# BVE-Reborn/rend3

Hardware: NVIDIA H100
Metric: culled objects/s (fused frustum cull + object-uniform bake) (higher is better)
Workload: dtype f32

## Files before the change

### include/rend3_b200.h

```cpp
#ifndef REND3_B200_H
#define REND3_B200_H

#include <stddef.h>
#include <stdint.h>

#include "r3_layouts.h"

#ifdef __cplusplus
extern "C" {
#endif

#define R3_ABI_VERSION 1u
#define R3_MAX_SHADOWS 63u

enum {
    R3_OK = 0,
    R3_E_INVALID = -1,
    R3_E_CUDA = -2,
    R3_E_OOM = -3,
    R3_E_NO_DEVICE = -4,
    R3_E_STATE = -5
};

typedef struct r3_ctx r3_ctx;

uint32_t r3_abi_version(void);
int r3_ctx_create(int device, r3_ctx** out);
int r3_ctx_destroy(r3_ctx* ctx);
const char* r3_last_error(const r3_ctx* ctx);
int r3_sync(r3_ctx* ctx);
int r3_get_stream(r3_ctx* ctx, void** stream);
int r3_launch_count(r3_ctx* ctx, uint64_t* launches);

int r3_frame_begin(r3_ctx* ctx);
int r3_frame_end(r3_ctx* ctx);
int r3_frame_graph_stats(r3_ctx* ctx, uint64_t stats[4]);

int r3_set_stage_timing(r3_ctx* ctx, int enabled);
int r3_stage_times(r3_ctx* ctx, double ms[8], uint32_t launches[8]);

int r3_set_objects(r3_ctx*, const r3_object* records, uint32_t n_slots);
int r3_update_objects(r3_ctx*, const uint32_t* slots, const r3_object* records, uint32_t n);
int r3_set_objects_device(r3_ctx*, const void* device_records, uint32_t n_slots);
int r3_set_object_sort_info(r3_ctx*, const uint64_t* material_key, const uint8_t* flags,
                            const float* location_xyz, uint32_t n_slots);
int r3_update_object_sort_info(r3_ctx*, const uint32_t* slots, const uint64_t* material_key, const uint8_t* flags,
                               const float* location_xyz, uint32_t n);
int r3_resize_objects(r3_ctx*, uint32_t n_slots);
int r3_set_object_mesh_spheres(r3_ctx*, const uint32_t* slots_or_null, const float* center_radius , uint32_t n);
int r3_set_object_transforms(r3_ctx*, const uint32_t* slots_or_null, const float* mat4s , uint32_t n);
int r3_set_object_transforms_device(r3_ctx*, const uint32_t* d_slots_or_null, const float* d_mat4s, uint32_t n);
int r3_set_objects_enabled(r3_ctx*, const uint32_t* slots_or_null, const uint8_t* enabled, uint32_t n);
int r3_set_objects_enabled_device(r3_ctx*, const uint32_t* d_slots_or_null, const uint8_t* d_enabled, uint32_t n);
int r3_set_object_variants(r3_ctx*, const r3_object_variant* variants, uint32_t n_variants, const r3_variant_group* groups, uint32_t n_groups,
                           const uint32_t* slots, const uint32_t* slot_groups, uint32_t n_listed);
int r3_switch_object_variants(r3_ctx*, const uint32_t* slots_or_null, const uint32_t* choices, uint32_t n);
int r3_switch_object_variants_device(r3_ctx*, const uint32_t* d_slots_or_null, const uint32_t* d_choices, uint32_t n);
int r3_readback_object_variants(r3_ctx*, uint32_t* out, uint32_t first, uint32_t n);
int r3_set_mesh_buffer(r3_ctx*, const void* bytes, uint64_t nbytes);
int r3_set_deformable_meshes(r3_ctx*, const r3_deformable_mesh* meshes, uint32_t n_meshes,
                             const uint32_t* object_slots, const uint32_t* object_meshes, uint32_t n_objects);
int r3_deform_meshes(r3_ctx*, const float* positions, uint64_t n_floats);
int r3_deform_meshes_device(r3_ctx*, const float* d_positions, uint64_t n_floats);
int r3_readback_deformable_mesh_spheres(r3_ctx*, float* out , uint32_t first, uint32_t n);
int r3_set_remeshable_meshes(r3_ctx*, const r3_remeshable_mesh* meshes, uint32_t n_meshes,
                             const uint32_t* object_slots, const uint32_t* object_meshes, uint32_t n_objects);
int r3_remesh_meshes(r3_ctx*, const uint32_t* counts, const float* positions, const uint32_t* indices, const float* normals,
                     const float* tangents, const float* uv0, const uint32_t* color0, uint64_t n_vertices, uint64_t n_indices);
int r3_remesh_meshes_device(r3_ctx*, const uint32_t* d_counts, const float* d_positions, const uint32_t* d_indices, const float* d_normals,
// ... 126 lines not shown
```

### include/rend3_b200.hpp

```cpp
#ifndef REND3_B200_HPP
#define REND3_B200_HPP

#include <array>
#include <cstdint>
#include <stdexcept>
#include <string>
#include <vector>

#include "rend3_b200.h"

namespace r3 {

struct Error : std::runtime_error {
    int code;
    Error(int c, const std::string& what) : std::runtime_error(what), code(c) {}
};

enum class SampleCount : uint32_t { One = 1, Four = 4 };
enum class CullingSource { Predicted, Residual };

struct CameraSpecifier {
    uint32_t index;
    static CameraSpecifier Viewport() { return {R3_CAMERA_VIEWPORT}; }
    static CameraSpecifier Shadow(uint32_t i) { return {i}; }
// ... 136 lines not shown
class HiZRoutine {
public:
    void add_hi_z_to_graph(Renderer& r) const { r.check(r3_hiz_build(r.raw())); }
};

class TonemappingRoutine {
public:
    void add_to_graph(Renderer& r, bool target_is_srgb) const { r.check(r3_tonemap(r.raw(), target_is_srgb ? 1 : 0)); }
};

class BaseRenderGraph {
public:
    GpuCuller gpu_culler;
    GpuSkinner gpu_skinner;
    ForwardRoutine forward;
    HiZRoutine hi_z;
    TonemappingRoutine tonemapping;
    bool submit_as_graph = false;
    bool device_shadow_cameras = false;
    bool device_point_lights = false;

    void add_to_graph(Renderer& r, const EvalOutput& ev, uint32_t width, uint32_t height, SampleCount samples, const BaseRenderGraphSettings& settings,
                      bool target_is_srgb = true) {
        r.check(r3_set_render_target(r.raw(), width, height, (uint32_t)samples, settings.clear_color.data()));
        if (submit_as_graph) r.check(r3_frame_begin(r.raw()));
        r.check(r3_clear_shadow_atlas(r.raw()));
        r.check(r3_set_frame_uniforms(r.raw(), &ev.uniforms));
        if (device_shadow_cameras) r.check(r3_evaluate_shadow_cameras(r.raw(), ev.viewport_location));
        if (device_point_lights) r.check(r3_evaluate_point_lights(r.raw()));
        if (ev.n_material_updates) r.check(r3_update_materials(r.raw(), ev.material_indices, ev.material_records, ev.n_material_updates));
        if (ev.n_d_material_updates) r.check(r3_update_materials_device(r.raw(), ev.d_material_indices, ev.d_material_records, ev.n_d_material_updates));
        gpu_skinner.add_skinning_to_graph(r, ev);
        for (uint32_t i = 0; i < ev.shadows.size(); ++i) {
            if (device_shadow_cameras) r.check(r3_shadow_uniform_upload(r.raw(), i, ev.n_slots, R3_CB_BAKE | R3_CB_CULL));
            else gpu_culler.object_uniform_upload(r, CameraSpecifier::Shadow(i), ev.shadows[i].header);
        }
        for (uint32_t i = 0; i < ev.shadows.size(); ++i) gpu_culler.add_culling_to_graph(r, CameraSpecifier::Shadow(i), ev.viewport_location);
        for (uint32_t i = 0; i < ev.shadows.size(); ++i) forward.add_shadow_to_graph(r, i, ev.shadows[i]);
        gpu_culler.object_uniform_upload(r, CameraSpecifier::Viewport(), ev.viewport);
        r.check(r3_forward_begin(r.raw()));
        forward.add_forward_to_graph(r, CullingSource::Predicted);
        hi_z.add_hi_z_to_graph(r);
        gpu_culler.add_culling_to_graph(r, CameraSpecifier::Viewport(), ev.viewport_location);
        forward.add_forward_to_graph(r, CullingSource::Residual);
        forward.resolve(r);
        forward.add_transparent_to_graph(r);
        tonemapping.add_to_graph(r, target_is_srgb);
        if (submit_as_graph) r.check(r3_frame_end(r.raw()));
    }
};

}
#endif
```

### rend3_b200/backend.py

```python
from __future__ import annotations

import ctypes as C
import os
from typing import Optional

import numpy as np

from .layouts import (
    BATCH_DTYPE,
    CAMERA_HEADER_DTYPE,
    INDIRECT_CALL_DTYPE,
    OBJECT_MATRICES_DTYPE,
    REGION_DTYPE,
)

CAMERA_VIEWPORT = 0xFFFFFFFF
CB_BAKE, CB_CULL = 1, 2

_ROOT = os.path.dirname(os.path.abspath(__file__))
CUDA_LIB_PATH = os.path.join(_ROOT, "librend3_b200.so")

ENTRY_POINTS = [
    "abi_version", "ctx_create", "ctx_destroy", "last_error", "sync", "get_stream", "launch_count", "set_stage_timing", "stage_times", "frame_begin", "frame_end", "frame_graph_stats",
    "set_objects", "update_objects", "set_objects_device", "set_object_sort_info", "set_mesh_buffer", "set_textures", "set_skybox",
    "set_materials", "set_directional_lights", "set_point_lights", "set_frame_uniforms",
    "object_uniform_upload", "visible_count", "readback_visible", "readback_object_matrices",
    "batch_objects", "batch_counts", "readback_batches", "batching_info", "cull", "readback_indices",
    "readback_draw_calls", "readback_culling_results", "set_render_target", "clear_shadow_atlas",
    "shadow_pass", "forward_begin", "forward_pass", "hiz_build", "forward_resolve", "forward_blend", "tonemap",
    "set_parity_target", "readback_hdr_f32", "readback_hdr_f16", "readback_depth", "readback_ldr", "readback_shadow_atlas",
    "readback_hiz", "forward_stats", "forward_light_evaluations", "device_ptr", "set_scissor_rows", "skin", "readback_mesh_buffer",
    "exchange_create", "exchange_connect", "exchange_words", "exchange_merge", "exchange_merged", "exchange_count", "exchange_counts", "exchange_destroy",
    "peer_create", "peer_connect", "peer_send_atlas_rect", "peer_send_rows", "peer_signal", "peer_wait", "peer_destroy", "clear_shadow_rect", "set_cull_shard",
    "update_object_sort_info", "resize_objects", "update_mesh_buffer", "update_textures",
    "set_animations", "set_skeletons", "set_pose_jobs", "pose_skeletons", "skin_posed", "readback_joint_matrices",
    "set_object_animations", "set_object_pose_jobs", "pose_objects", "readback_objects",
    "set_object_mesh_spheres", "set_object_transforms", "set_object_transforms_device",
    "set_objects_enabled", "set_objects_enabled_device",
    "update_materials", "update_materials_device", "readback_materials",
    "set_joint_matrices", "set_joint_matrices_device",
    "set_deformable_meshes", "deform_meshes", "deform_meshes_device", "readback_deformable_mesh_spheres",
    "set_remeshable_meshes", "remesh_meshes", "remesh_meshes_device", "readback_remesh_status", "debug_invocation_bound",
    "set_object_variants", "switch_object_variants", "switch_object_variants_device", "readback_object_variants",
]


class _AnimLibrary(C.Structure):
    _fields_ = [("skins", C.c_void_p), ("n_skins", C.c_uint32), ("joints", C.c_void_p), ("n_joints", C.c_uint32), ("order", C.c_void_p),
                ("clips", C.c_void_p), ("n_clips", C.c_uint32), ("channels", C.c_void_p), ("n_channels", C.c_uint32),
                ("keys", C.c_void_p), ("n_keys", C.c_uint64)]


class _AnimObjectLibrary(C.Structure):
    _fields_ = [("nodes", C.c_void_p), ("n_nodes", C.c_uint32), ("clips", C.c_void_p), ("n_clips", C.c_uint32), ("channels", C.c_void_p),
                ("n_channels", C.c_uint32), ("keys", C.c_void_p), ("n_keys", C.c_uint64), ("left_handed", C.c_uint32)]


class R3Error(RuntimeError):
    def __init__(self, code: int, message: str):
        super().__init__(f"rend3_b200 error {code}: {message}")
        self.code = code


def _ptr(a: Optional[np.ndarray]):
    return None if a is None else a.ctypes.data_as(C.c_void_p)


def _u32_list(a, what: str) -> np.ndarray:
    a = np.asarray(a)
    assert a.ndim == 1 and a.dtype.kind in "iu", f"{what}: a 1-d integer array"
    assert not len(a) or (a.min() >= 0 and a.max() <= 0xFFFFFFFF), f"{what}: out of the uint32 range"
    return np.ascontiguousarray(a, dtype=np.uint32)


class Backend:

    def __init__(self, lib: C.CDLL, prefix: str = "r3_", device: int = 0):
        self.lib, self.prefix = lib, prefix
        self.ctx = C.c_void_p()
        self._fn("last_error").restype = C.c_char_p
        self._fn("abi_version").restype = C.c_uint32
        rc = self._fn("ctx_create")(C.c_int(device), C.byref(self.ctx))
        if rc != 0:
            raise R3Error(rc, "context creation failed (no CUDA device?)")

    def _fn(self, name):
        return getattr(self.lib, self.prefix + name)

    def _call(self, name, *args):
        rc = self._fn(name)(self.ctx, *args)
        if rc != 0:
            raise R3Error(rc, (self._fn("last_error")(self.ctx) or b"?").decode())

    def close(self):
        if self.ctx:
            self._fn("ctx_destroy")(self.ctx)
            self.ctx = C.c_void_p()

    def __del__(self):
        try:
            self.close()
        except Exception:
            pass

    def sync(self):
        self._call("sync")

    def stream(self) -> int:
        s = C.c_void_p()
        self._call("get_stream", C.byref(s))
        return s.value or 0

    def launch_count(self) -> int:
        n = C.c_uint64()
        self._call("launch_count", C.byref(n))
        return n.value

    STAGES = ("triangle_test", "raster_setup_colour", "raster_setup_depth", "raster_bands", "resolve", "sort", "cull_bake", "triangle_compact")

    def frame_begin(self):
        self._call("frame_begin")

    def frame_end(self):
        self._call("frame_end")

    def frame_graph_stats(self):
        s = (C.c_uint64 * 4)()
        self._call("frame_graph_stats", s)
        return {"frames": int(s[0]), "graphed": int(s[1]), "flushed": int(s[2]), "instantiations": int(s[3])}

    def set_stage_timing(self, enabled: bool = True):
        self._call("set_stage_timing", C.c_int(1 if enabled else 0))

    def stage_times(self):
        ms, n = (C.c_double * 8)(), (C.c_uint32 * 8)()
        self._call("stage_times", ms, n)
        return {name: {"ms": float(ms[i]), "launches": int(n[i])} for i, name in enumerate(self.STAGES)}

    def set_objects(self, records: np.ndarray):
        records = np.ascontiguousarray(records)
        assert records.dtype.itemsize == 128
        self._call("set_objects", _ptr(records), C.c_uint32(len(records)))

    def set_objects_device(self, device_ptr: int, n_slots: int):
        self._call("set_objects_device", C.c_void_p(device_ptr), C.c_uint32(n_slots))

    def update_objects(self, slots: np.ndarray, records: np.ndarray):
        slots = np.ascontiguousarray(slots, dtype=np.uint32)
        records = np.ascontiguousarray(records)
        self._call("update_objects", _ptr(slots), _ptr(records), C.c_uint32(len(slots)))

    def set_object_sort_info(self, material_key, flags, location):
        k = np.ascontiguousarray(material_key, dtype=np.uint64)
        f = np.ascontiguousarray(flags, dtype=np.uint8)
        l = np.ascontiguousarray(location, dtype=np.float32).reshape(-1)
        assert len(f) == len(k) and len(l) == 3 * len(k)
        self._call("set_object_sort_info", _ptr(k), _ptr(f), _ptr(l), C.c_uint32(len(k)))
# ... 664 lines not shown
```

### rend3_b200/csrc/r3_common.cuh

```cuda
#pragma once
#include <cuda_runtime.h>
#include <stdint.h>

#include <string>
#include <vector>

#include "../../include/rend3_b200.h"

#define R3_EXPORT extern "C" __attribute__((visibility("default")))

constexpr int R3_MAX_CAMERAS = 64;

struct r3_iobuf {
    uint8_t* d = nullptr;
    uint64_t capacity_elements = 0, out_elems = 0, in_elems = 0, elem_size = 0;
    bool flipped = false, clear_on_swap = false, created = false;
    uint64_t out_off() const { return flipped ? capacity_elements / 2 : 0; }
    uint64_t in_off() const { return flipped ? 0 : capacity_elements / 2; }
};

struct r3_jobs {
    r3_batch_data* d_batches = nullptr; uint32_t batches_cap = 0, n_batches = 0;
    r3_region* d_regions = nullptr; uint32_t regions_cap = 0, n_regions = 0;
    uint32_t* d_region_first_inv = nullptr;
    uint32_t* d_header = nullptr;
    uint32_t total_invocations = 0;
    bool device_built = false;
    std::vector<r3_batch_data> batches;
    std::vector<r3_region> regions;
    bool valid = false;
};

enum { R3_STAGE_TRIANGLE_TEST = 0, R3_STAGE_RASTER_SETUP_COLOUR, R3_STAGE_RASTER_SETUP_DEPTH, R3_STAGE_RASTER_BANDS, R3_STAGE_RESOLVE, R3_STAGE_SORT,
       R3_STAGE_CULL_BAKE, R3_STAGE_TRIANGLE_COMPACT, R3_STAGE_COUNT };
struct r3_stage_timer {
    bool enabled = false;
    std::vector<cudaEvent_t> pool;
    std::vector<int> stage_of;
    size_t used = 0;
};
constexpr int R3_MAX_EXCHANGE_RANKS = 16;
constexpr int R3_EXCHANGE_SLOTS = 4;
constexpr uint32_t R3_PEER_KINDS = 4;
struct r3_peer_state {
// ... 9 lines not shown
struct r3_camera {
    bool header_set = false;
    r3_camera_header header{};
    r3_object_matrices* d_matrices = nullptr; uint32_t matrices_cap = 0;
    uint32_t* d_visible = nullptr; uint32_t visible_cap = 0;
    uint32_t* d_visible_count = nullptr;
    unsigned long long* d_tile_state = nullptr; uint32_t tile_state_cap = 0;
    uint32_t* d_words = nullptr; uint32_t words_set = 0;
    uint32_t* d_gathered = nullptr; uint32_t ex_ranks = 0, ex_rank = 0, ex_words_per_rank = 0; bool ex_connected = false;
    uint32_t* ex_peers[R3_MAX_EXCHANGE_RANKS] = {};
    uint32_t ex_epoch = 0, ex_objects = 0; uint32_t* d_ex_done = nullptr;
    cudaEvent_t ex_cull_done[R3_EXCHANGE_SLOTS] = {}, ex_merge_done[R3_EXCHANGE_SLOTS] = {}; bool ex_merge_pending[R3_EXCHANGE_SLOTS] = {}; uint32_t ex_consumed[R3_EXCHANGE_SLOTS] = {};
    uint32_t* d_global_visible = nullptr; uint64_t global_visible_cap = 0; uint32_t* d_merge_counts = nullptr; uint64_t merge_counts_cap = 0;
    int visible_count_host = -1;
    r3_jobs jobs[2]; int cur = 0;
    int batching_path = 0;
    uint64_t gsort_epoch_used = ~0ull;
    bool has_draw_call_set = false; int cache_idx = -1;
    std::vector<uint32_t> prev_invocation;
    uint32_t* d_prev_inv[2] = {nullptr, nullptr}; uint32_t prev_inv_cap = 0; int prev_inv_cur = 0;
    unsigned long long* d_sort_keys[2] = {nullptr, nullptr}; uint64_t sort_keys_cap = 0, sort_keys_cap2 = 0;
    uint32_t* d_sort_hist = nullptr; uint64_t sort_hist_cap = 0;
    uint32_t* d_batch_tmp = nullptr; uint64_t batch_tmp_cap = 0;
    r3_iobuf index_buffer, draw_call_buffer, results_buffer;
    uint32_t* d_resid_bits = nullptr; uint64_t resid_bits_cap = 0;
    unsigned long long* d_word_scan = nullptr; uint64_t word_scan_cap = 0;
    unsigned long long* d_block_sums = nullptr; uint64_t block_sums_cap = 0;
};

struct r3_anim_state;
struct r3_deform_state;
struct r3_variant_state;

struct r3_tri_record { float xyw[3][3]; uint32_t object_id; uint32_t vid[3]; uint32_t _pad[3]; };
static_assert(sizeof(r3_tri_record) == 64, "triangle record");

struct r3_ctx {
    int device = 0;
    cudaStream_t stream = nullptr;
    cudaStream_t side_stream = nullptr;
    std::string err;
    uint64_t launches = 0;
    bool coop_launch_ok = false;
    int sm_count = 1;
    r3_object* d_objects = nullptr; uint32_t n_slots = 0, objects_cap = 0; bool objects_borrowed = false;
    float4* d_hot_xyz = nullptr; float4* d_hot_w = nullptr; float4* d_hot_sphere = nullptr; uint32_t* d_enabled_bits = nullptr; uint32_t* d_affine_bits = nullptr;
    float* d_hot_radius = nullptr; uint32_t* d_centre_bits = nullptr;
    uint64_t hot_cap = 0; bool hot_valid = false;
    std::vector<uint64_t> sort_key; std::vector<uint8_t> sort_flags; std::vector<float> sort_loc;
    uint32_t* d_live_bits = nullptr; uint32_t live_bits_cap = 0; bool have_live = false;
    uint8_t* d_sort_key8 = nullptr; float* d_sort_loc = nullptr; uint32_t sort_dev_cap = 0; bool gpu_batching_ok = false;
    float4* d_mesh_spheres = nullptr; uint32_t n_mesh_spheres = 0, mesh_spheres_cap = 0;
    bool locations_moved = false;
    uint32_t sort_live_blend = 0, sort_wide_keys = 0;
    uint32_t sort_blend_slots = 0;
    bool presence_on_device = false;
    bool variants_on_device = false, variant_key2 = false, variant_wide_key = false;
    unsigned long long* d_gsort_keys[2] = {nullptr, nullptr}; uint64_t gsort_cap[2] = {0, 0}; uint32_t* d_gsort_hist = nullptr; uint64_t gsort_hist_cap = 0;
    uint32_t* d_gsort_header = nullptr; int gsort_src = 0; uint32_t gsort_n = 0; bool gsort_valid = false; float gsort_loc[3] = {0, 0, 0};
    uint64_t gsort_epoch = 0, gsort_sorted_epoch = ~0ull; uint32_t gsort_cameras_this_epoch = 0, gsort_cameras_last_epoch = 0;
    uint64_t max_total_invocations = 0, max_object_invocations = 0; bool max_invocations_valid = false;
    uint32_t* d_invocation_floor = nullptr; uint32_t n_invocation_floor = 0, invocation_floor_cap = 0;
    uint32_t* d_mesh = nullptr; uint64_t mesh_words = 0, mesh_cap = 0;
    r3_material* d_materials = nullptr; uint32_t n_materials = 0, materials_cap = 0;
    bool has_skybox = false; r3_texture_desc sky_desc{}; uint8_t* d_sky_texels = nullptr; uint64_t sky_cap = 0;
    r3_texture_desc* d_tex_descs = nullptr; uint32_t n_textures = 0, tex_descs_cap = 0; uint8_t* d_texels = nullptr; uint64_t texels_cap = 0, texel_bytes = 0;
    r3_directional_light* d_dir = nullptr; uint32_t n_dir = 0, dir_cap = 0;
    r3_directional_light_source* d_light_src = nullptr; r3_camera_header* d_shadow_cams = nullptr;
    std::vector<r3_directional_light_source> light_src;
    bool light_src_set = false, shadow_cams_evaluated = false; uint32_t light_src_left_handed = 0;
    uint8_t* d_point = nullptr; uint64_t point_bytes_cap = 0; uint32_t point_capacity = 0;
    r3_point_light_source* d_point_src = nullptr; uint8_t* d_point_live = nullptr; uint32_t point_handles = 0, point_src_cap = 0, point_live_cap = 0;
// ... 156 lines not shown
```

### rend3_b200/csrc/r3_ctx.cu

```cuda
#include <algorithm>
#include <cstdio>
#include <cstdlib>
#include <cstring>
#include <new>

#include "r3_common.cuh"

int r3_fail(r3_ctx* c, int code, const char* msg) {
    if (c) c->err = msg;
    return code;
}
int r3_cuda_fail(r3_ctx* c, cudaError_t e, const char* where) {
    if (c) {
        c->err = std::string(where) + ": " + cudaGetErrorString(e);
    }
    cudaGetLastError();
    return e == cudaErrorMemoryAllocation ? R3_E_OOM : R3_E_CUDA;
}

int r3_reserve(r3_ctx* c, void** ptr, uint64_t* cap, uint64_t need, size_t elem, bool keep, bool zero_new) {
    if (*ptr && *cap >= need) return R3_OK;
    uint64_t ncap = need < 16 ? 16 : need;
    void* n = nullptr;
    R3_CUDA(c, cudaMalloc(&n, ncap * elem));
    if (zero_new) R3_CUDA(c, cudaMemsetAsync(n, 0, ncap * elem, c->stream));
    if (*ptr) {
        if (keep && *cap) R3_CUDA(c, cudaMemcpyAsync(n, *ptr, *cap * elem, cudaMemcpyDeviceToDevice, c->stream));
        R3_CUDA(c, r3_stream_sync(c));
        cudaFree(*ptr);
    }
    *ptr = n;
    *cap = ncap;
    return R3_OK;
}

R3_EXPORT uint32_t r3_abi_version(void) { return R3_ABI_VERSION; }

R3_EXPORT int r3_ctx_create(int device, r3_ctx** out) {
    if (!out) return R3_E_INVALID;
    *out = nullptr;
    int count = 0;
    cudaError_t e = cudaGetDeviceCount(&count);
    if (e != cudaSuccess || count == 0 || device < 0 || device >= count) {
        cudaGetLastError();
        return R3_E_NO_DEVICE;
    }
    r3_ctx* c = new (std::nothrow) r3_ctx();
    if (!c) return R3_E_OOM;
    c->device = device;
    int prio_least = 0, prio_greatest = 0;
    if (cudaSetDevice(device) == cudaSuccess) cudaDeviceGetStreamPriorityRange(&prio_least, &prio_greatest);
    if (cudaSetDevice(device) != cudaSuccess || cudaStreamCreateWithPriority(&c->stream, cudaStreamNonBlocking, prio_greatest) != cudaSuccess) {
        delete c;
        cudaGetLastError();
        return R3_E_CUDA;
    }
    { int coop = 0; cudaDeviceGetAttribute(&coop, cudaDevAttrCooperativeLaunch, device); c->coop_launch_ok = coop != 0; }
    if (cudaDeviceGetAttribute(&c->sm_count, cudaDevAttrMultiProcessorCount, device) != cudaSuccess || c->sm_count < 1) { cudaStreamDestroy(c->stream); delete c; cudaGetLastError(); return R3_E_CUDA; }
    if (cudaMalloc((void**)&c->d_stats, 8 * sizeof(unsigned long long)) != cudaSuccess) { delete c; return R3_E_OOM; }
    cudaMemsetAsync(c->d_stats, 0, 64, c->stream);
    c->point_bytes_cap = 16 + 16 * sizeof(r3_point_light);
    if (cudaMalloc((void**)&c->d_point, c->point_bytes_cap) != cudaSuccess) { cudaFree(c->d_stats); delete c; return R3_E_OOM; }
    cudaMemsetAsync(c->d_point, 0, c->point_bytes_cap, c->stream);
    *out = c;
    return R3_OK;
}

static void free_jobs(r3_jobs& j) { cudaFree(j.d_batches); cudaFree(j.d_regions); cudaFree(j.d_region_first_inv); cudaFree(j.d_header); }

R3_EXPORT int r3_ctx_destroy(r3_ctx* c) {
    if (!c) return R3_E_INVALID;
    cudaSetDevice(c->device);
    r3_stream_sync(c);
    if (c->side_stream) cudaStreamSynchronize(c->side_stream);
    r3_peer_destroy(c);
    r3_anim_destroy(c);
    r3_deform_destroy(c);
    r3_variants_destroy(c);
    if (!c->objects_borrowed) cudaFree(c->d_objects);
    cudaFree(c->d_hot_xyz); cudaFree(c->d_hot_w); cudaFree(c->d_hot_sphere); cudaFree(c->d_enabled_bits); cudaFree(c->d_affine_bits); cudaFree(c->d_hot_radius); cudaFree(c->d_centre_bits); cudaFree(c->d_tex_descs); cudaFree(c->d_texels); cudaFree(c->d_sky_texels);
    cudaFree(c->d_sort_key8); cudaFree(c->d_sort_loc); cudaFree(c->d_gsort_keys[0]); cudaFree(c->d_gsort_keys[1]); cudaFree(c->d_gsort_hist); cudaFree(c->d_gsort_header);
    cudaFree(c->d_mesh_spheres); cudaFree(c->d_live_bits); cudaFree(c->d_mesh); cudaFree(c->d_materials); cudaFree(c->d_dir); cudaFree(c->d_point);
    cudaFree(c->d_light_mats); cudaFree(c->d_atlas); cudaFree(c->d_light_src); cudaFree(c->d_shadow_cams); cudaFree(c->d_point_src); cudaFree(c->d_point_live);
    for (auto& k : c->cams) {
        cudaFree(k.d_matrices); cudaFree(k.d_visible); cudaFree(k.d_visible_count); cudaFree(k.d_tile_state);
        if (k.d_gathered) {
            for (uint32_t r = 0; r < k.ex_ranks; ++r)
                if (k.ex_connected && r != k.ex_rank && k.ex_peers[r]) cudaIpcCloseMemHandle(k.ex_peers[r]);
            cudaFree(k.d_gathered);
        }
        cudaFree(k.d_ex_done); cudaFree(k.d_global_visible); cudaFree(k.d_merge_counts);
        for (int q = 0; q < R3_EXCHANGE_SLOTS; ++q) { if (k.ex_cull_done[q]) cudaEventDestroy(k.ex_cull_done[q]); if (k.ex_merge_done[q]) cudaEventDestroy(k.ex_merge_done[q]); }
        free_jobs(k.jobs[0]); free_jobs(k.jobs[1]);
        cudaFree(k.index_buffer.d); cudaFree(k.draw_call_buffer.d); cudaFree(k.results_buffer.d);
        cudaFree(k.d_resid_bits); cudaFree(k.d_word_scan); cudaFree(k.d_block_sums);
        cudaFree(k.d_prev_inv[0]); cudaFree(k.d_prev_inv[1]); cudaFree(k.d_sort_keys[0]); cudaFree(k.d_sort_keys[1]); cudaFree(k.d_sort_hist); cudaFree(k.d_batch_tmp);
    }
    cudaFree(c->d_vis); cudaFree(c->d_hdr32); cudaFree(c->d_hdr16); cudaFree(c->d_depth); cudaFree(c->d_ldr);
    for (float* p : c->d_hiz) cudaFree(p);
    cudaFree(c->d_hiz_ptrs); cudaFree(c->d_hiz_dims);
    cudaFree(c->d_tris[0]); cudaFree(c->d_tris[1]); cudaFree(c->d_tris[2]); cudaFree(c->d_tris[3]); cudaFree(c->d_stats); cudaFree(c->d_scratch);
    cudaFree(c->d_frag_heads); cudaFree(c->d_frag_nodes);
    for (cudaEvent_t e : c->timer.pool) cudaEventDestroy(e);
    for (auto& x : c->frame_exec) if (x) cudaGraphExecDestroy(x);
    if (c->side_stream) cudaStreamDestroy(c->side_stream);
    cudaStreamDestroy(c->stream);
    delete c;
    return R3_OK;
}
R3_EXPORT const char* r3_last_error(const r3_ctx* c) { return c ? c->err.c_str() : "null context"; }
R3_EXPORT int r3_sync(r3_ctx* c) {
    if (!c) return R3_E_INVALID;
    cudaSetDevice(c->device);
    R3_CUDA(c, r3_stream_sync(c));
    if (c->side_stream) R3_CUDA(c, cudaStreamSynchronize(c->side_stream));
    return R3_OK;
}
R3_EXPORT int r3_get_stream(r3_ctx* c, void** s) {
    if (!c || !s) return R3_E_INVALID;
    *s = (void*)c->stream;
    return R3_OK;
}
R3_EXPORT int r3_launch_count(r3_ctx* c, uint64_t* n) {
    if (!c || !n) return R3_E_INVALID;
    *n = c->launches;
    return R3_OK;
}

static cudaError_t r3_submit_capture(r3_ctx* c, int slot) {
    if (!c->capturing) return cudaSuccess;
    c->capturing = false;
    cudaGraph_t g = nullptr;
    cudaError_t e = cudaStreamEndCapture(c->stream, &g);
    if (e != cudaSuccess || !g) return e != cudaSuccess ? e : cudaErrorUnknown;
    if (slot < 0) {
        cudaGraphExec_t x = nullptr;
        e = cudaGraphInstantiate(&x, g, 0);
        if (e == cudaSuccess) e = cudaGraphLaunch(x, c->stream);
        if (e == cudaSuccess) e = cudaStreamSynchronize(c->stream);
        if (x) cudaGraphExecDestroy(x);
        cudaGraphDestroy(g);
        return e;
    }
    cudaGraphExec_t& x = c->frame_exec[slot];
    if (x) {
        cudaGraphExecUpdateResultInfo info;
        if (cudaGraphExecUpdate(x, g, &info) != cudaSuccess) {
            cudaGetLastError();
            cudaGraphExecDestroy(x);
            x = nullptr;
        }
    }
    if (!x) {
        e = cudaGraphInstantiate(&x, g, 0);
        c->graph_reinstantiations++;
    }
    if (e == cudaSuccess) e = cudaGraphLaunch(x, c->stream);
    cudaGraphDestroy(g);
    return e;
}
cudaError_t r3_stream_sync(r3_ctx* c) {
    if (c->capturing) {
        const cudaError_t e = r3_submit_capture(c, -1);
        c->frames_flushed++;
        if (e != cudaSuccess) return e;
    }
    return cudaStreamSynchronize(c->stream);
}
R3_EXPORT int r3_frame_begin(r3_ctx* c) {
    if (!c) return R3_E_INVALID;
    cudaSetDevice(c->device);
    if (c->capturing) return r3_fail(c, R3_E_STATE, "frame_begin: a frame is already being recorded");
    if (c->timer.enabled) return R3_OK;
    if (c->gpu_batching_ok) R3_TRY(r3_compute_max_invocations(c));
    R3_CUDA(c, cudaStreamBeginCapture(c->stream, cudaStreamCaptureModeRelaxed));
    c->capturing = true;
    return R3_OK;
}
R3_EXPORT int r3_frame_end(r3_ctx* c) {
    if (!c) return R3_E_INVALID;
    cudaSetDevice(c->device);
    const bool was = c->capturing;
    const cudaError_t e = r3_submit_capture(c, (int)(c->frame_index & 1u));
    c->frame_index++;
    if (was) c->frames_graphed++;
    if (e != cudaSuccess) return r3_cuda_fail(c, e, "frame_end (graph submission)");
    return R3_OK;
}
R3_EXPORT int r3_frame_graph_stats(r3_ctx* c, uint64_t stats[4]) {
    if (!c || !stats) return R3_E_INVALID;
    stats[0] = c->frame_index; stats[1] = c->frames_graphed; stats[2] = c->frames_flushed; stats[3] = c->graph_reinstantiations;
    return R3_OK;
}

void r3_stage_begin(r3_ctx* c, int stage) {
    r3_stage_timer& t = c->timer;
    if (!t.enabled || c->capturing) return;
    if (t.pool.size() < 2 * (t.used + 1)) {
        cudaEvent_t a = nullptr, b = nullptr;
        if (cudaEventCreate(&a) != cudaSuccess || cudaEventCreate(&b) != cudaSuccess) { t.enabled = false; return; }
        t.pool.push_back(a); t.pool.push_back(b); t.stage_of.push_back(stage);
    }
    t.stage_of[t.used] = stage;
    cudaEventRecord(t.pool[2 * t.used], c->stream);
}
void r3_stage_end(r3_ctx* c) {
    r3_stage_timer& t = c->timer;
    if (!t.enabled || c->capturing) return;
    cudaEventRecord(t.pool[2 * t.used + 1], c->stream);
    t.used++;
}
R3_EXPORT int r3_set_stage_timing(r3_ctx* c, int enabled) {
    if (!c) return R3_E_INVALID;
    cudaSetDevice(c->device);
// ... 727 lines not shown
```

### rend3_b200/csrc/r3_gpu_batching.cu

```cuda
#include <algorithm>
#include <cstring>

#include <cooperative_groups.h>
#include <cuda/atomic>

#include "r3_common.cuh"
#include "r3_radix.cuh"
#include "r3_scan.cuh"

namespace {

constexpr int KEY_SHIFT0 = 24, SORT_PASSES = 5;

__device__ __forceinline__ uint32_t sortable_f32(float f) {
    if (f != f) return 0xFFC00000u;
    const uint32_t b = __float_as_uint(f) == 0x80000000u ? 0u : __float_as_uint(f);
    return (b & 0x80000000u) ? ~b : (b | 0x80000000u);
}

__device__ __forceinline__ unsigned long long make_sort_key(const uint32_t* __restrict__ visible, const uint8_t* __restrict__ key8, const float* __restrict__ loc,
                                                            float vx, float vy, float vz, uint32_t j) {
    const uint32_t h = visible ? visible[j] : j;
    const uint8_t k = key8[h];
    const float dx = sub_rn(vx, loc[3 * (size_t)h]), dy = sub_rn(vy, loc[3 * (size_t)h + 1]), dz = sub_rn(vz, loc[3 * (size_t)h + 2]);
// ... 433 lines not shown
        c->launches++;
        src = SORT_PASSES & 1;
    } else {
        keygen_kernel<<<(cap + 255) / 256, 256, 0, c->stream>>>(visible, visible_count, c->d_sort_key8, c->d_sort_loc, vp_loc[0], vp_loc[1], vp_loc[2], keys[0], header, cap);
        R3_CHECK_LAUNCH(c, "keygen_kernel");
        for (int pass = 0; pass < SORT_PASSES; ++pass) {
            const int shift = KEY_SHIFT0 + 8 * pass;
            radix_hist_kernel<<<sort_blocks, SORT_THREADS, 0, c->stream>>>(keys[src], header, shift, *hist);
            R3_CHECK_LAUNCH(c, "radix_hist_kernel");
            scan_u32_kernel<<<1, 1024, 0, c->stream>>>(*hist, sort_blocks * 256u);
            R3_CHECK_LAUNCH(c, "scan_u32_kernel");
            radix_scatter_kernel<<<sort_blocks, SORT_THREADS, 0, c->stream>>>(keys[src], keys[src ^ 1], header, shift, *hist);
            R3_CHECK_LAUNCH(c, "radix_scatter_kernel");
            src ^= 1;
        }
    }
    r3_stage_end(c);
    *src_out = src;
    return R3_OK;
}

static bool r3_frame_sort_wanted(r3_ctx* c, r3_camera* cam, const float vp_loc[3]) {
    if (cam->gsort_epoch_used == c->gsort_epoch || (c->gsort_cameras_this_epoch > 0 && memcmp(c->gsort_loc, vp_loc, 12) != 0)) r3_new_frame_epoch(c);
    if (c->gsort_cameras_this_epoch == 0) memcpy(c->gsort_loc, vp_loc, 12);
    cam->gsort_epoch_used = c->gsort_epoch;
    c->gsort_cameras_this_epoch++;
    const char* force = getenv("R3_FRAME_SORT");
    if (force) return force[0] != '0';
    if (c->n_slots > (1u << 22)) return false;
    return c->gsort_cameras_last_epoch >= 2 || (c->gsort_cameras_last_epoch == 0 && c->n_dir >= 1);
}
static int r3_frame_sort(r3_ctx* c, const float vp_loc[3]) {
    if (c->gsort_valid && c->gsort_sorted_epoch == c->gsort_epoch) return R3_OK;
    const uint32_t n = (uint32_t)(c->sort_flags.size() < c->n_slots ? c->sort_flags.size() : c->n_slots);
    R3_TRY(r3_reserve_t(c, &c->d_gsort_keys[0], &c->gsort_cap[0], (uint64_t)n + 1));
    R3_TRY(r3_reserve_t(c, &c->d_gsort_keys[1], &c->gsort_cap[1], (uint64_t)n + 1));
    if (!c->d_gsort_header) R3_CUDA(c, cudaMalloc((void**)&c->d_gsort_header, 32));
    int src = 0;
    if (n) R3_TRY(r3_launch_sort(c, nullptr, nullptr, n, vp_loc, c->d_gsort_keys, &c->d_gsort_hist, &c->gsort_hist_cap, c->d_gsort_header, &src));
    c->gsort_src = src; c->gsort_n = n; c->gsort_valid = true; c->gsort_sorted_epoch = c->gsort_epoch;
    return R3_OK;
}

int r3_device_batch_objects(r3_ctx* c, r3_camera* cam, const float vp_loc[3], uint32_t max_dispatch_count) {
    if (!cam->header_set) return r3_fail(c, R3_E_STATE, "batch_objects before object_uniform_upload");
    const uint32_t cap = cam->header.object_count;
    R3_TRY(r3_compute_max_invocations(c));
    if (c->max_total_invocations >= (1ull << 31)) return r3_fail(c, R3_E_INVALID, "more than 2^31 padded invocations");
    const int w = (cam->cache_idx == 0) ? 1 : 0;
    cam->cur = w;
    r3_jobs& j = cam->jobs[w];
    const uint64_t dispatch_limit = (uint64_t)max_dispatch_count * R3_WORKGROUP_SIZE;
    const bool partition = c->max_object_invocations * R3_BATCH_SIZE >= dispatch_limit;
    uint64_t nb_max = (cap + 255u) / 256u;
    if (partition) {
        nb_max = (uint64_t)cap + 1u;
        if (dispatch_limit) nb_max = std::min<uint64_t>(nb_max, (cap + 255u) / 256u + 2u * (c->max_total_invocations / dispatch_limit) + 3u);
    }
    const uint32_t nb_cap = (uint32_t)nb_max + 1u, nr_cap = nb_cap + 64u;
    R3_TRY(r3_reserve_t(c, &j.d_batches, &j.batches_cap, nb_cap));
    uint32_t rcap = j.regions_cap;
    R3_TRY(r3_reserve_t(c, &j.d_regions, &j.regions_cap, nr_cap));
    if (!j.d_region_first_inv || rcap != j.regions_cap) {
        cudaFree(j.d_region_first_inv);
        j.d_region_first_inv = nullptr;
        R3_CUDA(c, cudaMalloc((void**)&j.d_region_first_inv, ((size_t)j.regions_cap + 2) * 4));
    }
    if (!j.d_header) R3_CUDA(c, cudaMalloc((void**)&j.d_header, 32));
    R3_TRY(r3_reserve_t(c, &cam->d_sort_keys[0], &cam->sort_keys_cap, (uint64_t)cap + 1));
    R3_TRY(r3_reserve_t(c, &cam->d_sort_keys[1], &cam->sort_keys_cap2, (uint64_t)cap + 1));
    const uint32_t sort_blocks = (cap + SORT_TILE - 1) / SORT_TILE;
    R3_TRY(r3_reserve_t(c, &cam->d_sort_hist, &cam->sort_hist_cap, (uint64_t)sort_blocks * 256 + 1));
    const uint32_t part_tiles = (cap + 255u) / 256u, mark_tiles = (cap + 1023u) / 1024u;
// ... 109 lines not shown
```

### rend3_b200/routines.py

```python
from __future__ import annotations

from dataclasses import dataclass
from typing import Optional, Tuple

import numpy as np

from . import glam
from .backend import CAMERA_VIEWPORT, CB_BAKE, CB_CULL, Backend
from .layouts import CAMERA_HEADER_DTYPE, FRAME_UNIFORMS_DTYPE, PCU_MULTISAMPLED, PCU_POSITIVE_AREA_VISIBLE
from .world import LEFT, CameraState, EvalOutput, frustum_from_matrix

f32 = np.float32


def triangle_visibility_positive(handedness: str, shadow: bool) -> bool:
    cw = handedness == LEFT
    front_culled = shadow
    return (not cw and not front_culled) or (cw and front_culled)


def per_camera_header(camera: CameraState, camera_specifier: int, resolution: Tuple[int, int], samples: int,
                      object_count: int) -> np.ndarray:
    h = np.zeros((), dtype=CAMERA_HEADER_DTYPE)
    h["view"] = camera.view.reshape(16)
    h["view_proj"] = camera.view_proj.reshape(16)
    h["shadow_index"] = camera_specifier
    h["frustum"] = camera.world_frustum
    h["resolution"] = np.array(resolution, dtype=f32)
    flags = 0
    if triangle_visibility_positive(camera.handedness, camera_specifier != CAMERA_VIEWPORT):
        flags |= PCU_POSITIVE_AREA_VISIBLE
    if samples != 1:
        flags |= PCU_MULTISAMPLED
    h["flags"] = flags
    h["object_count"] = object_count
    return h


def frame_uniforms(camera: CameraState, ambient, resolution: Tuple[int, int]) -> np.ndarray:
    u = np.zeros((), dtype=FRAME_UNIFORMS_DTYPE)
    u["view"] = camera.view.reshape(16)
# ... 124 lines not shown
            else:
                b.update_materials(records, indices)
        if object_variants is not None:
            slots, choices = object_variants
            if getattr(choices, "is_cuda", False):
                b.switch_object_variants_device(choices, slots)
            else:
                b.switch_object_variants(choices, slots)
        if object_presence is not None:
            slots, enabled = object_presence
            if getattr(enabled, "is_cuda", False):
                b.set_objects_enabled_device(enabled, slots)
            else:
                b.set_objects_enabled(enabled, slots)
        if object_transforms is not None:
            slots, matrices = object_transforms
            if getattr(matrices, "is_cuda", False):
                b.set_object_transforms_device(matrices, slots)
            else:
                b.set_object_transforms(matrices, slots)
        if posed_objects:
            b.pose_objects()
        if posed_skinning:
            b.pose_skeletons()
        if joint_matrices is not None:
            writes, mat4s, inverse_binds = joint_matrices
            if getattr(mat4s, "is_cuda", False):
                b.set_joint_matrices_device(writes, mat4s, inverse_binds)
            else:
                b.set_joint_matrices(writes, mat4s, inverse_binds)
        if posed_skinning or joint_matrices is not None:
            b.skin_posed()
        mine = [(i, s) for i, s in enumerate(ev.shadows) if shadow_filter is None or shadow_filter(i)]
        for i, s in mine:
            if device_shadow_cameras:
                b.shadow_uniform_upload(i, len(ev.object_buffer))
            else:
                culler.object_uniform_upload(ev, s.camera, i, (s.size, s.size), 1)
        for i, s in mine:
            culler.cull(ev, i)
        for i, s in mine:
            b.shadow_pass(i, s.offset[0], s.offset[1], s.size)
        if after_shadows is not None:
            after_shadows()
        culler.object_uniform_upload(ev, ev.camera, CAMERA_VIEWPORT, resolution, samples)
        b.forward_begin()
        b.forward_pass(0)
        b.hiz_build()
        culler.cull(ev, CAMERA_VIEWPORT)
        b.forward_pass(1)
        if before_resolve is not None:
            before_resolve()
        b.forward_resolve()
        b.forward_blend()
        if tonemap:
            b.tonemap(srgb_target)
        if frame_graph:
            b.frame_end()
```

Measured before the change: 14.84 billion.

## Run per-shadow cull and render chains on forked branch streams

Adds branch streams with fork/join events so each shadow camera's upload, cull and shadow pass run as an independent chain on one of four side streams, concurrent with the viewport chain on the main stream. Per-branch scratch and triangle buffers are swapped in so concurrent chains do not share temporaries, and the global sort is forced back onto the main stream. This targets serialization across cameras but adds event and stream overhead and the risk of hidden data hazards between branches.

New measurement: 14.79 billion, median of 6. No clear change (-0.3%).

```diff
diff --git a/include/rend3_b200.h b/include/rend3_b200.h
--- a/include/rend3_b200.h
+++ b/include/rend3_b200.h
@@ -35,6 +35,11 @@
 int r3_frame_begin(r3_ctx* ctx);
 int r3_frame_end(r3_ctx* ctx);
 int r3_frame_graph_stats(r3_ctx* ctx, uint64_t stats[4]);
+
+#define R3_MAX_BRANCHES 4u
+#define R3_BRANCH_MAIN (-1)
+int r3_branch_begin(r3_ctx* ctx, int branch);
+int r3_branch_join(r3_ctx* ctx);
 
 int r3_set_stage_timing(r3_ctx* ctx, int enabled);
 int r3_stage_times(r3_ctx* ctx, double ms[8], uint32_t launches[8]);
diff --git a/include/rend3_b200.hpp b/include/rend3_b200.hpp
--- a/include/rend3_b200.hpp
+++ b/include/rend3_b200.hpp
@@ -192,17 +192,20 @@
         if (ev.n_d_material_updates) r.check(r3_update_materials_device(r.raw(), ev.d_material_indices, ev.d_material_records, ev.n_d_material_updates));
         gpu_skinner.add_skinning_to_graph(r, ev);
         for (uint32_t i = 0; i < ev.shadows.size(); ++i) {
+            r.check(r3_branch_begin(r.raw(), (int)(i % R3_MAX_BRANCHES)));
             if (device_shadow_cameras) r.check(r3_shadow_uniform_upload(r.raw(), i, ev.n_slots, R3_CB_BAKE | R3_CB_CULL));
             else gpu_culler.object_uniform_upload(r, CameraSpecifier::Shadow(i), ev.shadows[i].header);
+            gpu_culler.add_culling_to_graph(r, CameraSpecifier::Shadow(i), ev.viewport_location);
+            forward.add_shadow_to_graph(r, i, ev.shadows[i]);
         }
-        for (uint32_t i = 0; i < ev.shadows.size(); ++i) gpu_culler.add_culling_to_graph(r, CameraSpecifier::Shadow(i), ev.viewport_location);
-        for (uint32_t i = 0; i < ev.shadows.size(); ++i) forward.add_shadow_to_graph(r, i, ev.shadows[i]);
+        r.check(r3_branch_begin(r.raw(), R3_BRANCH_MAIN));
         gpu_culler.object_uniform_upload(r, CameraSpecifier::Viewport(), ev.viewport);
         r.check(r3_forward_begin(r.raw()));
         forward.add_forward_to_graph(r, CullingSource::Predicted);
         hi_z.add_hi_z_to_graph(r);
         gpu_culler.add_culling_to_graph(r, CameraSpecifier::Viewport(), ev.viewport_location);
         forward.add_forward_to_graph(r, CullingSource::Residual);
+        r.check(r3_branch_join(r.raw()));
         forward.resolve(r);
         forward.add_transparent_to_graph(r);
         tonemapping.add_to_graph(r, target_is_srgb);
diff --git a/rend3_b200/backend.py b/rend3_b200/backend.py
--- a/rend3_b200/backend.py
+++ b/rend3_b200/backend.py
@@ -16,12 +16,14 @@
 
 CAMERA_VIEWPORT = 0xFFFFFFFF
 CB_BAKE, CB_CULL = 1, 2
+MAX_BRANCHES, BRANCH_MAIN = 4, -1
 
 _ROOT = os.path.dirname(os.path.abspath(__file__))
 CUDA_LIB_PATH = os.path.join(_ROOT, "librend3_b200.so")
 
 ENTRY_POINTS = [
     "abi_version", "ctx_create", "ctx_destroy", "last_error", "sync", "get_stream", "launch_count", "set_stage_timing", "stage_times", "frame_begin", "frame_end", "frame_graph_stats",
+    "branch_begin", "branch_join",
     "set_objects", "update_objects", "set_objects_device", "set_object_sort_info", "set_mesh_buffer", "set_textures", "set_skybox",
     "set_materials", "set_directional_lights", "set_point_lights", "set_frame_uniforms",
     "object_uniform_upload", "visible_count", "readback_visible", "readback_object_matrices",
@@ -73,6 +75,20 @@
     return np.ascontiguousarray(a, dtype=np.uint32)
 
 
+class Branches:
+
+    def __init__(self, backend: "Backend"):
+        self.backend = backend
+
+    def begin(self, branch: int):
+        if self.backend._has_branches:
+            self.backend._call("branch_begin", C.c_int(branch))
+
+    def join(self):
+        if self.backend._has_branches:
+            self.backend._call("branch_join")
+
+
 class Backend:
 
     def __init__(self, lib: C.CDLL, prefix: str = "r3_", device: int = 0):
@@ -80,6 +96,7 @@
         self.ctx = C.c_void_p()
         self._fn("last_error").restype = C.c_char_p
         self._fn("abi_version").restype = C.c_uint32
+        self._has_branches = hasattr(lib, prefix + "branch_begin")
         rc = self._fn("ctx_create")(C.c_int(device), C.byref(self.ctx))
         if rc != 0:
             raise R3Error(rc, "context creation failed (no CUDA device?)")
@@ -123,6 +140,10 @@
 
     def frame_end(self):
         self._call("frame_end")
+
+    @property
+    def branches(self) -> "Branches":
+        return Branches(self)
 
     def frame_graph_stats(self):
         s = (C.c_uint64 * 4)()
diff --git a/rend3_b200/csrc/r3_common.cuh b/rend3_b200/csrc/r3_common.cuh
--- a/rend3_b200/csrc/r3_common.cuh
+++ b/rend3_b200/csrc/r3_common.cuh
@@ -10,6 +10,9 @@
 #define R3_EXPORT extern "C" __attribute__((visibility("default")))
 
 constexpr int R3_MAX_CAMERAS = 64;
+
+struct r3_tri_record { float xyw[3][3]; uint32_t object_id; uint32_t vid[3]; uint32_t _pad[3]; };
+static_assert(sizeof(r3_tri_record) == 64, "triangle record");
 
 struct r3_iobuf {
     uint8_t* d = nullptr;
@@ -85,12 +88,20 @@
 struct r3_deform_state;
 struct r3_variant_state;
 
-struct r3_tri_record { float xyw[3][3]; uint32_t object_id; uint32_t vid[3]; uint32_t _pad[3]; };
-static_assert(sizeof(r3_tri_record) == 64, "triangle record");
+struct r3_branch {
+    cudaStream_t stream = nullptr;
+    cudaEvent_t fork = nullptr, join = nullptr;
+    bool open = false;
+    void* d_scratch = nullptr; uint64_t scratch_cap = 0;
+    r3_tri_record* d_tris = nullptr; uint64_t tris_cap = 0;
+};
 
 struct r3_ctx {
     int device = 0;
     cudaStream_t stream = nullptr;
+    cudaStream_t main_stream = nullptr;
+    r3_branch branches[R3_MAX_BRANCHES];
+    int branch = R3_BRANCH_MAIN;
     cudaStream_t side_stream = nullptr;
     std::string err;
     uint64_t launches = 0;
diff --git a/rend3_b200/csrc/r3_ctx.cu b/rend3_b200/csrc/r3_ctx.cu
--- a/rend3_b200/csrc/r3_ctx.cu
+++ b/rend3_b200/csrc/r3_ctx.cu
@@ -55,12 +55,20 @@
         cudaGetLastError();
         return R3_E_CUDA;
     }
+    c->main_stream = c->stream;
+    for (r3_branch& b : c->branches)
+        if (cudaStreamCreateWithPriority(&b.stream, cudaStreamNonBlocking, prio_greatest) != cudaSuccess ||
+            cudaEventCreateWithFlags(&b.fork, cudaEventDisableTiming) != cudaSuccess || cudaEventCreateWithFlags(&b.join, cudaEventDisableTiming) != cudaSuccess) {
+            cudaGetLastError();
+            r3_ctx_destroy(c);
+            return R3_E_CUDA;
+        }
     { int coop = 0; cudaDeviceGetAttribute(&coop, cudaDevAttrCooperativeLaunch, device); c->coop_launch_ok = coop != 0; }
-    if (cudaDeviceGetAttribute(&c->sm_count, cudaDevAttrMultiProcessorCount, device) != cudaSuccess || c->sm_count < 1) { cudaStreamDestroy(c->stream); delete c; cudaGetLastError(); return R3_E_CUDA; }
-    if (cudaMalloc((void**)&c->d_stats, 8 * sizeof(unsigned long long)) != cudaSuccess) { delete c; return R3_E_OOM; }
+    if (cudaDeviceGetAttribute(&c->sm_count, cudaDevAttrMultiProcessorCount, device) != cudaSuccess || c->sm_count < 1) { cudaGetLastError(); r3_ctx_destroy(c); return R3_E_CUDA; }
+    if (cudaMalloc((void**)&c->d_stats, 8 * sizeof(unsigned long long)) != cudaSuccess) { cudaGetLastError(); r3_ctx_destroy(c); return R3_E_OOM; }
     cudaMemsetAsync(c->d_stats, 0, 64, c->stream);
     c->point_bytes_cap = 16 + 16 * sizeof(r3_point_light);
-    if (cudaMalloc((void**)&c->d_point, c->point_bytes_cap) != cudaSuccess) { cudaFree(c->d_stats); delete c; return R3_E_OOM; }
+    if (cudaMalloc((void**)&c->d_point, c->point_bytes_cap) != cudaSuccess) { cudaGetLastError(); r3_ctx_destroy(c); return R3_E_OOM; }
     cudaMemsetAsync(c->d_point, 0, c->point_bytes_cap, c->stream);
     *out = c;
     return R3_OK;
@@ -72,6 +80,7 @@
     if (!c) return R3_E_INVALID;
     cudaSetDevice(c->device);
     r3_stream_sync(c);
+    r3_branch_join(c);
     if (c->side_stream) cudaStreamSynchronize(c->side_stream);
     r3_peer_destroy(c);
     r3_anim_destroy(c);
@@ -104,7 +113,13 @@
     for (cudaEvent_t e : c->timer.pool) cudaEventDestroy(e);
     for (auto& x : c->frame_exec) if (x) cudaGraphExecDestroy(x);
     if (c->side_stream) cudaStreamDestroy(c->side_stream);
-    cudaStreamDestroy(c->stream);
+    for (r3_branch& b : c->branches) {
+        cudaFree(b.d_scratch); cudaFree(b.d_tris);
+        if (b.fork) cudaEventDestroy(b.fork);
+        if (b.join) cudaEventDestroy(b.join);
+        if (b.stream) cudaStreamDestroy(b.stream);
+    }
+    cudaStreamDestroy(c->main_stream);
     delete c;
     return R3_OK;
 }
@@ -118,7 +133,7 @@
 }
 R3_EXPORT int r3_get_stream(r3_ctx* c, void** s) {
     if (!c || !s) return R3_E_INVALID;
-    *s = (void*)c->stream;
+    *s = (void*)c->main_stream;
     return R3_OK;
 }
 R3_EXPORT int r3_launch_count(r3_ctx* c, uint64_t* n) {
@@ -131,13 +146,13 @@
     if (!c->capturing) return cudaSuccess;
     c->capturing = false;
     cudaGraph_t g = nullptr;
-    cudaError_t e = cudaStreamEndCapture(c->stream, &g);
+    cudaError_t e = cudaStreamEndCapture(c->main_stream, &g);
     if (e != cudaSuccess || !g) return e != cudaSuccess ? e : cudaErrorUnknown;
     if (slot < 0) {
         cudaGraphExec_t x = nullptr;
         e = cudaGraphInstantiate(&x, g, 0);
-        if (e == cudaSuccess) e = cudaGraphLaunch(x, c->stream);
-        if (e == cudaSuccess) e = cudaStreamSynchronize(c->stream);
+        if (e == cudaSuccess) e = cudaGraphLaunch(x, c->main_stream);
+        if (e == cudaSuccess) e = cudaStreamSynchronize(c->main_stream);
         if (x) cudaGraphExecDestroy(x);
         cudaGraphDestroy(g);
         return e;
@@ -155,17 +170,66 @@
         e = cudaGraphInstantiate(&x, g, 0);
         c->graph_reinstantiations++;
     }
-    if (e == cudaSuccess) e = cudaGraphLaunch(x, c->stream);
+    if (e == cudaSuccess) e = cudaGraphLaunch(x, c->main_stream);
     cudaGraphDestroy(g);
     return e;
 }
+
+static void branch_switch(r3_ctx* c, int k) {
+    if (c->branch == k) return;
+    for (int s : {c->branch, k}) {
+        if (s < 0) continue;
+        r3_branch& b = c->branches[s];
+        std::swap(b.d_scratch, c->d_scratch); std::swap(b.scratch_cap, c->scratch_cap);
+        std::swap(b.d_tris, c->d_tris[3]); std::swap(b.tris_cap, c->tris_cap[3]);
+    }
+    c->branch = k;
+    c->stream = k < 0 ? c->main_stream : c->branches[k].stream;
+}
+static cudaError_t branch_fork(r3_ctx* c, r3_branch& b) {
+    cudaError_t e = cudaEventRecord(b.fork, c->main_stream);
+    if (e == cudaSuccess) e = cudaStreamWaitEvent(b.stream, b.fork, 0);
+    b.open = e == cudaSuccess;
+    return e;
+}
+static cudaError_t branch_join_all(r3_ctx* c) {
+    for (r3_branch& b : c->branches) {
+        if (!b.open) continue;
+        cudaError_t e = cudaEventRecord(b.join, b.stream);
+        if (e == cudaSuccess) e = cudaStreamWaitEvent(c->main_stream, b.join, 0);
+        if (e != cudaSuccess) return e;
+        b.open = false;
+    }
+    return cudaSuccess;
+}
+R3_EXPORT int r3_branch_begin(r3_ctx* c, int k) {
+    if (!c) return R3_E_INVALID;
+    if (k < R3_BRANCH_MAIN || k >= (int)R3_MAX_BRANCHES) return r3_fail(c, R3_E_INVALID, "branch_begin: no such branch");
+    if (c->timer.enabled) return R3_OK;
+    cudaSetDevice(c->device);
+    branch_switch(c, k);
+    if (k >= 0) R3_CUDA(c, branch_fork(c, c->branches[k]));
+    return R3_OK;
+}
+R3_EXPORT int r3_branch_join(r3_ctx* c) {
+    if (!c) return R3_E_INVALID;
+    cudaSetDevice(c->device);
+    branch_switch(c, R3_BRANCH_MAIN);
+    R3_CUDA(c, branch_join_all(c));
+    return R3_OK;
+}
+
 cudaError_t r3_stream_sync(r3_ctx* c) {
+    cudaError_t e = branch_join_all(c);
+    if (e != cudaSuccess) return e;
     if (c->capturing) {
-        const cudaError_t e = r3_submit_capture(c, -1);
+        e = r3_submit_capture(c, -1);
         c->frames_flushed++;
         if (e != cudaSuccess) return e;
     }
-    return cudaStreamSynchronize(c->stream);
+    e = cudaStreamSynchronize(c->main_stream);
+    if (e == cudaSuccess && c->branch >= 0) e = branch_fork(c, c->branches[c->branch]);
+    return e;
 }
 R3_EXPORT int r3_frame_begin(r3_ctx* c) {
     if (!c) return R3_E_INVALID;
@@ -173,13 +237,15 @@
     if (c->capturing) return r3_fail(c, R3_E_STATE, "frame_begin: a frame is already being recorded");
     if (c->timer.enabled) return R3_OK;
     if (c->gpu_batching_ok) R3_TRY(r3_compute_max_invocations(c));
-    R3_CUDA(c, cudaStreamBeginCapture(c->stream, cudaStreamCaptureModeRelaxed));
+    R3_TRY(r3_branch_join(c));
+    R3_CUDA(c, cudaStreamBeginCapture(c->main_stream, cudaStreamCaptureModeRelaxed));
     c->capturing = true;
     return R3_OK;
 }
 R3_EXPORT int r3_frame_end(r3_ctx* c) {
     if (!c) return R3_E_INVALID;
     cudaSetDevice(c->device);
+    R3_TRY(r3_branch_join(c));
     const bool was = c->capturing;
     const cudaError_t e = r3_submit_capture(c, (int)(c->frame_index & 1u));
     c->frame_index++;
diff --git a/rend3_b200/csrc/r3_gpu_batching.cu b/rend3_b200/csrc/r3_gpu_batching.cu
--- a/rend3_b200/csrc/r3_gpu_batching.cu
+++ b/rend3_b200/csrc/r3_gpu_batching.cu
@@ -489,6 +489,8 @@
 }
 static int r3_frame_sort(r3_ctx* c, const float vp_loc[3]) {
     if (c->gsort_valid && c->gsort_sorted_epoch == c->gsort_epoch) return R3_OK;
+    const int branch = c->branch;
+    if (branch >= 0) R3_TRY(r3_branch_begin(c, R3_BRANCH_MAIN));
     const uint32_t n = (uint32_t)(c->sort_flags.size() < c->n_slots ? c->sort_flags.size() : c->n_slots);
     R3_TRY(r3_reserve_t(c, &c->d_gsort_keys[0], &c->gsort_cap[0], (uint64_t)n + 1));
     R3_TRY(r3_reserve_t(c, &c->d_gsort_keys[1], &c->gsort_cap[1], (uint64_t)n + 1));
@@ -496,6 +498,7 @@
     int src = 0;
     if (n) R3_TRY(r3_launch_sort(c, nullptr, nullptr, n, vp_loc, c->d_gsort_keys, &c->d_gsort_hist, &c->gsort_hist_cap, c->d_gsort_header, &src));
     c->gsort_src = src; c->gsort_n = n; c->gsort_valid = true; c->gsort_sorted_epoch = c->gsort_epoch;
+    if (branch >= 0) R3_TRY(r3_branch_begin(c, branch));
     return R3_OK;
 }
 
diff --git a/rend3_b200/routines.py b/rend3_b200/routines.py
--- a/rend3_b200/routines.py
+++ b/rend3_b200/routines.py
@@ -6,7 +6,7 @@
 import numpy as np
 
 from . import glam
-from .backend import CAMERA_VIEWPORT, CB_BAKE, CB_CULL, Backend
+from .backend import BRANCH_MAIN, CAMERA_VIEWPORT, CB_BAKE, CB_CULL, MAX_BRANCHES, Backend
 from .layouts import CAMERA_HEADER_DTYPE, FRAME_UNIFORMS_DTYPE, PCU_MULTISAMPLED, PCU_POSITIVE_AREA_VISIBLE
 from .world import LEFT, CameraState, EvalOutput, frustum_from_matrix
 
@@ -197,23 +197,27 @@
         if posed_skinning or joint_matrices is not None:
             b.skin_posed()
         mine = [(i, s) for i, s in enumerate(ev.shadows) if shadow_filter is None or shadow_filter(i)]
-        for i, s in mine:
+        branches = b.branches
+        for n, (i, s) in enumerate(mine):
+            branches.begin(n % MAX_BRANCHES)
             if device_shadow_cameras:
                 b.shadow_uniform_upload(i, len(ev.object_buffer))
             else:
                 culler.object_uniform_upload(ev, s.camera, i, (s.size, s.size), 1)
-        for i, s in mine:
             culler.cull(ev, i)
-        for i, s in mine:
             b.shadow_pass(i, s.offset[0], s.offset[1], s.size)
         if after_shadows is not None:
+            branches.join()
             after_shadows()
+        else:
+            branches.begin(BRANCH_MAIN)
         culler.object_uniform_upload(ev, ev.camera, CAMERA_VIEWPORT, resolution, samples)
         b.forward_begin()
         b.forward_pass(0)
         b.hiz_build()
         culler.cull(ev, CAMERA_VIEWPORT)
         b.forward_pass(1)
+        branches.join()
         if before_resolve is not None:
             before_resolve()
         b.forward_resolve()
```
